# InternetMaximalism/plonky2_bn254

Hardware: AMD Instinct MI355X
Metric: G1 scalar-mul STARK proofs/sec (256-bit scalars) (higher is better)
Workload: dtype u64 (Goldilocks p = 2^64-2^32+1; BN254 Fq as 10x26-bit Montgomery limbs); 1 GPU; configs[1]: batch of 1024 G1 scalar-muls on 1 GPU per step = 8 proofs x 128 instances, 2^16 rows, W=781, standard_fast_config; instances_per_proof=128, steps_in_flight=4, parallelism=1 GPU, no collective

## Files before the change

### plonky2_bn254_amd/csrc/quotient_common.h

```cpp
#pragma once
#include "gl_dev.h"
#include "aux.h"

struct Acc {
  u64 lo, hi;
  u32 ov;
};
__device__ __forceinline__ void acc_init(Acc& a) {
  a.lo = 0;
  a.hi = 0;
  a.ov = 0;
}
__device__ __forceinline__ void acc_mad(Acc& a, u64 x, u64 w) {
  const unsigned __int128 pr = (unsigned __int128)x * w;
  u64 pl = (u64)pr, ph = (u64)(pr >> 64);
  a.lo += pl;
  u64 c = a.lo < pl ? 1 : 0;
  u64 h = a.hi + ph;
  u32 o = h < ph ? 1 : 0;
  h += c;
  o += h < c ? 1 : 0;
  a.hi = h;
  a.ov += o;
}
__device__ __forceinline__ u64 acc_red(const Acc& a) {
  return gl_sub(gl_reduce128(a.lo, a.hi), ((u64)a.ov) << 32);
}
struct Acc2 {
  Acc a0, a1;
};
__device__ __forceinline__ void acc2_init(Acc2& a) {
  acc_init(a.a0);
  acc_init(a.a1);
}
__device__ __forceinline__ void acc2_mad(Acc2& a, u64 x, u64 w0, u64 w1) {
  acc_mad(a.a0, x, w0);
  acc_mad(a.a1, x, w1);
}

static constexpr u32 M22 = (1u << 22) - 1;
struct W3 {
  u32 w0, w1, w2;
};
GL_HD W3 w3_split(u64 w) {
  W3 r;
  r.w0 = (u32)w & M22;
  r.w1 = (u32)(w >> 22) & M22;
  r.w2 = (u32)(w >> 44);
  return r;
}
struct Acc3 {
  u64 c[5];
};
__device__ __forceinline__ void acc3_init(Acc3& a) {
#pragma unroll
  for (int k = 0; k < 5; k++) a.c[k] = 0;
}
__device__ __forceinline__ void acc3_mad(Acc3& a, u32 v0, u32 v1, u32 v2, u32 w0, u32 w1, u32 w2) {
  a.c[0] += (u64)v0 * w0;
  a.c[1] += (u64)v0 * w1;
  a.c[1] += (u64)v1 * w0;
  a.c[2] += (u64)v0 * w2;
  a.c[2] += (u64)v1 * w1;
  a.c[2] += (u64)v2 * w0;
  a.c[3] += (u64)v1 * w2;
  a.c[3] += (u64)v2 * w1;
  a.c[4] += (u64)v2 * w2;
}
__device__ __forceinline__ u64 acc3_red(const Acc3& a) {
  unsigned __int128 t = (unsigned __int128)a.c[0] + ((unsigned __int128)a.c[1] << 22) + ((unsigned __int128)a.c[2] << 44);
  u64 r = gl_reduce128((u64)t, (u64)(t >> 64));
  r = gl_add(r, gl_mul_2exp<66>(gl_reduce128(a.c[3], 0)));
  r = gl_add(r, gl_mul_2exp<88>(gl_reduce128(a.c[4], 0)));
  return r;
}

struct AccW {
  Acc3 a0, a1;
};
__device__ __forceinline__ void accw_init(AccW& a) {
  acc3_init(a.a0);
  acc3_init(a.a1);
}
template <class WP>
__device__ __forceinline__ void accw_mad(AccW& a, u64 x, WP w) {
  const u32 v0 = (u32)x & M22, v1 = (u32)(x >> 22) & M22, v2 = (u32)(x >> 44);
  acc3_mad(a.a0, v0, v1, v2, w[0], w[1], w[2]);
  acc3_mad(a.a1, v0, v1, v2, w[4], w[5], w[6]);
}
GL_HD void w3_store(u64* dst , u64 wa, u64 wb) {
  const W3 a = w3_split(wa), b = w3_split(wb);
  dst[0] = (u64)a.w0 | ((u64)a.w1 << 32);
  dst[1] = (u64)a.w2;
  dst[2] = (u64)b.w0 | ((u64)b.w1 << 32);
  dst[3] = (u64)b.w2;
}

struct QPointTables {
  const u64* x;
  const u64* lfirst;
  const u64* llast;
};

__device__ __forceinline__ size_t next_position(size_t j, unsigned log_n) {
  const size_t N = (size_t)1 << log_n;
  size_t h = j >> log_n;
  u32 k = bitrev32((u32)(j & (N - 1)), log_n);
  k = (k + 1) & (u32)(N - 1);
  return (h << log_n) | bitrev32(k, log_n);
}

__device__ __forceinline__ void lookup_and_ctl_constraints(const StarkShape& sh, const u64* __restrict__ tl,
                                                           const u64* __restrict__ al, size_t M2, size_t j, size_t jn,
                                                           const u32* __restrict__ W3 , int e0,
                                                           const u64 betas[2], const u64 gammas[2], u64 lfirst, u64 llast,
                                                           u64 z_last, u64& tot0, u64& tot1) {
  const int m = sh.n_helpers(), n_rc = sh.n_rc();
  int e = e0;
  AccW acc;
  accw_init(acc);
  const u64 table = tl[(size_t)sh.table_col * M2 + j], freq = tl[(size_t)sh.freq_col * M2 + j];
  u64 hs[2] = {0, 0};
#pragma unroll 4
  for (int k = 0; k < m; k++) {
    u64 f0 = tl[(size_t)(sh.rc_begin + 2 * k) * M2 + j];
    bool two = (2 * k + 1) < n_rc;
    u64 f1 = two ? tl[(size_t)(sh.rc_begin + 2 * k + 1) * M2 + j] : 0;
#pragma unroll
    for (int ch = 0; ch < 2; ch++) {
      u64 h = al[(size_t)(ch * (m + 1) + k) * M2 + j];
      u64 g0 = gl_add(f0, betas[ch]);
      u64 c;
      if (two) {
        u64 g1 = gl_add(f1, betas[ch]);
        c = gl_sub(gl_sub(gl_mul(gl_mul(g1, g0), h), g1), g0);
      } else {
        c = gl_sub(gl_mul(g0, h), 1);
      }
      int ee = e0 + ch * (m + 2) + k;
      accw_mad(acc, c, W3 + 8 * (ee));
      hs[ch] = gl_add(hs[ch], h);
    }
  }
#pragma unroll
  for (int ch = 0; ch < 2; ch++) {
    u64 z = al[(size_t)(ch * (m + 1) + m) * M2 + j], nz = al[(size_t)(ch * (m + 1) + m) * M2 + jn];
    u64 twc = gl_add(table, betas[ch]);
    u64 y = gl_sub(gl_mul(hs[ch], twc), freq);
    int ee = e0 + ch * (m + 2) + m;
    accw_mad(acc, gl_mul(z, lfirst), W3 + 8 * (ee));
    accw_mad(acc, gl_sub(gl_mul(gl_sub(nz, z), twc), y), W3 + 8 * (ee + 1));
  }
  e = e0 + 2 * (m + 2);
  for (int ctl = 0; ctl < sh.n_ctl; ctl++) {
    u64 a0 = 0, a1 = 0;
    for (int mm = sh.ctl.ncols[ctl] - 1; mm >= 0; mm--) {
      int start = sh.ctl.col_start[ctl][mm], nb = sh.ctl.col_bits[ctl][mm];
      u64 v = 0;
      for (int b = nb - 1; b >= 0; b--) v = gl_add(gl_dbl(v), tl[(size_t)(start + b) * M2 + j]);
      a0 = gl_add(gl_mul(a0, betas[0]), v);
      a1 = gl_add(gl_mul(a1, betas[1]), v);
    }
    u64 comb[2] = {gl_add(a0, gammas[0]), gl_add(a1, gammas[1])};
    u64 f0 = tl[(size_t)sh.ctl.filter_col[ctl] * M2 + j];
#pragma unroll
    for (int ch = 0; ch < 2; ch++) {
      int zc = 2 * (m + 1) + ctl * 2 + ch;
      u64 lz = al[(size_t)zc * M2 + j], nz = al[(size_t)zc * M2 + jn];
      u64 c_last = gl_mul(gl_sub(gl_mul(comb[ch], lz), f0), llast);
      u64 c_tr = gl_mul(gl_sub(gl_mul(comb[ch], gl_sub(lz, nz)), f0), z_last);
      accw_mad(acc, c_last, W3 + 8 * (e));
      accw_mad(acc, c_tr, W3 + 8 * (e + 1));
      e += 2;
    }
  }
  tot0 = gl_add(tot0, acc3_red(acc.a0));
  tot1 = gl_add(tot1, acc3_red(acc.a1));
}
```

### plonky2_bn254_amd/csrc/quotient_g1.hip

```cpp
#include "quotient_sched.h"
#include "trace_g1.h"
#include "quotient.h"

static constexpr int G1_K_AIR = 1111;
static constexpr int G1_MZ_E0[5] = {0, 50, 83, 132, 165};

template <int part>
__device__ __forceinline__ void g1_add_part(const QArgs& A, size_t j) {
  const size_t M2 = A.stride;
  const u64* __restrict__ tl = A.tl;
  const qc64 W0 = QCONST(u64, A.W);
  const qc64 W1 = QCONST(u64, A.W + A.K);
  const qc32 W3 = QCONST(u32, A.W + 2 * (size_t)A.K);
  u64 tot0 = 0, tot1 = 0;
  int e = 0;
  const int AUX = G1_COL_AUX;
  const u64 filter = TL(G1_COL_FILTER);
  const u64 is_x_eq_filter = TL(AUX + G1_AUX_IS_X_EQ_FILTER);
  u64 ax[16], lam[16], t16[16], u16[16];
  ld16(tl, M2, j, G1_COL_A, ax);
  if constexpr (part == 0) {
    const u64 is_x_eq = TL(AUX + G1_AUX_IS_X_EQ);
    ld16(tl, M2, j, G1_COL_B, u16);
#pragma unroll
    for (int i = 0; i < 16; i++) u16[i] = gl_sub(u16[i], ax[i]);
    ld16(tl, M2, j, AUX + G1_AUX_IS_X_EQ_AUX, t16);
    const u64 c0 = gl_sub(is_x_eq, 1);
    mz_block<true>(tl, M2, j, AUX + G1_AUX_IS_X_EQ_AUX + 16, A, G1_MZ_E0[0], 0,
             filter, [&](int i) __attribute__((always_inline)) { u64 v = conv16<true>(u16, t16, i); return i == 0 ? gl_add(v, c0) : v; }, tot0, tot1);
    e = 33;
    AccW g;
    accw_init(g);
#pragma unroll
    for (int i = 0; i < 16; i++) accw_mad(g, u16[i], W3 + 8 * (e + i));
    e += 16;
    u64 f = gl_mul(filter, is_x_eq);
    tot0 = gl_add(tot0, gl_mul(f, acc3_red(g.a0)));
    tot1 = gl_add(tot1, gl_mul(f, acc3_red(g.a1)));
    EMIT(gl_sub(gl_mul(filter, is_x_eq), is_x_eq_filter));
  } else if constexpr (part == 1) {
    ld16(tl, M2, j, AUX + G1_AUX_LAMBDA, lam);
    ld16(tl, M2, j, G1_COL_B, u16);
#pragma unroll
    for (int i = 0; i < 16; i++) u16[i] = gl_sub(u16[i], ax[i]);
    ld16(tl, M2, j, G1_COL_B + 16, t16);
    ld16(tl, M2, j, G1_COL_A + 16, ax);
#pragma unroll
    for (int i = 0; i < 16; i++) t16[i] = gl_sub(t16[i], ax[i]);
    mz_block<true>(tl, M2, j, AUX + G1_AUX_LAMBDA_AUX, A, G1_MZ_E0[1], 1,
             gl_sub(filter, is_x_eq_filter),
             [&](int i) __attribute__((always_inline)) {
               u64 v = conv16<true>(lam, u16, i);
               return i < 16 ? gl_sub(v, t16[i < 16 ? i : 0]) : v;
             },
             tot0, tot1);
  } else if constexpr (part == 2) {
    ld16(tl, M2, j, AUX + G1_AUX_LAMBDA, lam);
    ld16(tl, M2, j, G1_COL_A + 16, u16);
    mz_block<true>(tl, M2, j, AUX + G1_AUX_LAMBDA_AUX, A, G1_MZ_E0[2], 2,
             is_x_eq_filter,
             [&](int i) __attribute__((always_inline)) {
               u64 ly = conv16<true>(lam, u16, i), xx = conv16<true>(ax, ax, i);
               return gl_sub(gl_dbl(ly), gl_add(gl_dbl(xx), xx));
             },
             tot0, tot1);
    e = 116;
    ld16(tl, M2, j, G1_COL_B + 16, t16);
    AccW g;
    accw_init(g);
#pragma unroll
    for (int i = 0; i < 16; i++) accw_mad(g, gl_sub(u16[i], t16[i]), W3 + 8 * (e + i));
    tot0 = gl_add(tot0, gl_mul(is_x_eq_filter, acc3_red(g.a0)));
    tot1 = gl_add(tot1, gl_mul(is_x_eq_filter, acc3_red(g.a1)));
  } else if constexpr (part == 3) {
    ld16(tl, M2, j, AUX + G1_AUX_LAMBDA, lam);
    ld16(tl, M2, j, G1_COL_B, t16);
    ld16(tl, M2, j, G1_COL_C, u16);
#pragma unroll
    for (int i = 0; i < 16; i++) ax[i] = gl_add(gl_add(ax[i], t16[i]), u16[i]);
    mz_block<true>(tl, M2, j, AUX + G1_AUX_X_AUX, A, G1_MZ_E0[3], 3, filter,
             [&](int i) __attribute__((always_inline)) {
               u64 v = conv16<true>(lam, lam, i);
               return i < 16 ? gl_sub(v, ax[i < 16 ? i : 0]) : v;
             },
             tot0, tot1);
  } else {
    ld16(tl, M2, j, AUX + G1_AUX_LAMBDA, lam);
    ld16(tl, M2, j, G1_COL_C, u16);
#pragma unroll
    for (int i = 0; i < 16; i++) u16[i] = gl_sub(u16[i], ax[i]);
    ld16(tl, M2, j, G1_COL_C + 16, t16);
    ld16(tl, M2, j, G1_COL_A + 16, ax);
#pragma unroll
    for (int i = 0; i < 16; i++) t16[i] = gl_add(t16[i], ax[i]);
    mz_block<true>(tl, M2, j, AUX + G1_AUX_Y_AUX, A, G1_MZ_E0[4], 4, filter,
             [&](int i) __attribute__((always_inline)) {
               u64 v = conv16<true>(lam, u16, i);
               return i < 16 ? gl_add(v, t16[i < 16 ? i : 0]) : v;
             },
             tot0, tot1);
  }
  store_part(A, part, j, tot0, tot1);
}

__global__ __launch_bounds__(256, 2) void k_quotient_g1_parts(QArgs A) {
  const size_t j = (size_t)blockIdx.x * blockDim.x + threadIdx.x;
  if (j >= A.count) return;
  switch (blockIdx.y) {
    case 0: schedule_part<G1L, false>(A, j, q_next(A, j), 198, 5); break;
    case 1: g1_add_part<0>(A, j); break;
    case 2: g1_add_part<1>(A, j); break;
    case 3: g1_add_part<2>(A, j); break;
    case 4: g1_add_part<3>(A, j); break;
    default: g1_add_part<4>(A, j); break;
  }
}

__global__ __launch_bounds__(256) void k_quotient_finish(QArgs A, StarkShape sh) {
  const size_t j = (size_t)blockIdx.x * blockDim.x + threadIdx.x;
  if (j >= A.count) return;
  finish_point(A, sh, j);
}
void quotient_finish_launch(const QArgs& A, const StarkShape& sh, hipStream_t st) {
  k_quotient_finish<<<(unsigned)((A.count + 255) / 256), 256, 0, st>>>(A, sh);
}

__global__ void k_point_tables(u64* x, u64* lfirst, u64* llast, unsigned log_n, u64 w_n, u64 w_2n) {
  const size_t N = (size_t)1 << log_n;
  size_t j = (size_t)blockIdx.x * blockDim.x + threadIdx.x;
  if (j >= 2 * N) return;
  size_t h = j >> log_n;
  u32 k = bitrev32((u32)(j & (N - 1)), log_n);
  u64 shift = h ? gl_mul(GL_GEN, w_2n) : GL_GEN;
  u64 xv = gl_mul(shift, gl_pow(w_n, k));
  u64 gn = gl_pow(GL_GEN, N);
  u64 zh = gl_sub(h ? gl_neg(gn) : gn, 1);
  u64 ninv = gl_inv((u64)N % GL_P);
  u64 winv = gl_inv(w_n);
  x[j] = xv;
  lfirst[j] = gl_mul(gl_mul(zh, ninv), gl_inv(gl_sub(xv, 1)));
  llast[j] = gl_mul(gl_mul(gl_mul(zh, ninv), winv), gl_inv(gl_sub(xv, winv)));
}

__global__ void k_point_tables_window(u64* x, u64* lfirst, u64* llast, unsigned log_n, u32 h, size_t k0, size_t count, u64 w_n,
                                      u64 w_2n) {
  const size_t N = (size_t)1 << log_n;
  size_t j = (size_t)blockIdx.x * blockDim.x + threadIdx.x;
  if (j >= count) return;
  const u64 k = (k0 + j) & (N - 1);
  u64 shift = h ? gl_mul(GL_GEN, w_2n) : GL_GEN;
  u64 xv = gl_mul(shift, gl_pow(w_n, k));
  u64 gn = gl_pow(GL_GEN, N);
  u64 zh = gl_sub(h ? gl_neg(gn) : gn, 1);
  u64 ninv = gl_inv((u64)N % GL_P);
  u64 winv = gl_inv(w_n);
  x[j] = xv;
  lfirst[j] = gl_mul(gl_mul(zh, ninv), gl_inv(gl_sub(xv, 1)));
  llast[j] = gl_mul(gl_mul(gl_mul(zh, ninv), winv), gl_inv(gl_sub(xv, winv)));
}
void quotient_point_tables_window(u64* d_x, u64* d_lfirst, u64* d_llast, unsigned log_n, int h, size_t k0, size_t count, hipStream_t st) {
  k_point_tables_window<<<(unsigned)((count + 255) / 256), 256, 0, st>>>(d_x, d_lfirst, d_llast, log_n, (u32)h, k0, count,
                                                                       gl_root_of_unity(log_n), gl_root_of_unity(log_n + 1));
}
void quotient_window_args(QArgs& A, const u64* d_tw, const u64* d_aw, const QPointTables& pt, u64* d_part, size_t stride, size_t count,
                          size_t k0, int h) {
  A.tl = d_tw;
  A.al = d_aw;
  A.pt = pt;
  A.part = d_part;
  A.stride = stride;
  A.count = count;
  A.k0 = k0;
  A.natural = 1;
  A.hsel = (u32)h;
}

void quotient_point_tables(u64* d_x, u64* d_lfirst, u64* d_llast, unsigned log_n, hipStream_t st) {
  size_t M2 = (size_t)2 << log_n;
  k_point_tables<<<(unsigned)((M2 + 255) / 256), 256, 0, st>>>(d_x, d_lfirst, d_llast, log_n, gl_root_of_unity(log_n),
                                                             gl_root_of_unity(log_n + 1));
}

void quotient_host_tables(int K, const u64 alphas[2], const int* mz_e0, int n_blocks, std::vector<u64>& W, std::vector<u64>& mzt) {
  W.assign(QUOTIENT_W_WORDS(K), 0);
  for (int a = 0; a < 2; a++) {
    u64 v = 1;
    for (int e = K - 1; e >= 0; e--) {
      W[(size_t)a * K + e] = v;
      v = gl_mul(v, alphas[a]);
    }
  }
  static const u64 MOD[16] = {64839, 55420, 35862, 15392, 51853, 26737, 27281, 38785,
                              22621, 33153, 17846, 47184, 41001, 57649, 20082, 12388};
  const u64 B = 1ULL << 16, OFF = 1ULL << 29;
  mzt.assign(QUOTIENT_MZT_WORDS, 0);
  for (int blk = 0; blk < n_blocks; blk++)
    for (int a = 0; a < 2; a++) {
      const u64* w = &W[(size_t)a * K + mz_e0[blk] + 1];
      u64* T = &mzt[(size_t)(blk * 2 + a) * 80];
      for (int jj = 0; jj < 17; jj++) {
        u64 s = 0;
        for (int t = 0; t < 16; t++)
          if (jj + t < 32) s = gl_add(s, gl_mul(w[jj + t], MOD[t]));
        T[jj] = s;
      }
      u64 usum = 0;
      for (int d = 0; d < 31; d++) {
        u64 u = gl_sub(w[d + 1], gl_mul(B, w[d]));
        T[17 + d] = u;
        T[48 + d] = gl_mul(B, u);
        usum = gl_add(usum, u);
      }
      T[79] = gl_mul(OFF, usum);
    }
  for (int e = 0; e < K; e++) w3_store(&W[2 * (size_t)K + 4 * (size_t)e], W[e], W[(size_t)K + e]);
  for (int blk = 0; blk < n_blocks; blk++)
    for (int t = 0; t < 80; t++)
      w3_store(&mzt[QUOTIENT_MZT3_OFF + (size_t)(blk * 80 + t) * 4], mzt[(size_t)(blk * 2) * 80 + t], mzt[(size_t)(blk * 2 + 1) * 80 + t]);
}

void quotient_fill_args(QArgs& A, const StarkShape& sh, const u64* d_tl, const u64* d_al, const u64* d_W, const u64* d_mzt,
                        const QPointTables& pt, const u64 betas[2], const u64 gammas[2], unsigned log_n, u64* d_out,
                        u64* d_part) {
  A.tl = d_tl;
  A.al = d_al;
  A.W = d_W;
  A.mzt = d_mzt;
  A.pt = pt;
  for (int i = 0; i < 2; i++) {
    A.betas[i] = betas[i];
    A.gammas[i] = gammas[i];
  }
  const size_t N = (size_t)1 << log_n;
  u64 gn = gl_pow(GL_GEN, N);
  A.zh_inv[0] = gl_inv(gl_sub(gn, 1));
  A.zh_inv[1] = gl_inv(gl_sub(gl_neg(gn), 1));
  A.w_inv = gl_inv(gl_root_of_unity(log_n));
  A.out = d_out;
  A.part = d_part;
  A.n_parts = 0;
  A.log_n = log_n;
  A.K = sh.n_total_constraints();
  A.stride = A.count = 2 * N;
  A.k0 = 0;
  A.natural = 0;
  A.hsel = 0;
}

int g1_quotient_mz_blocks(const int** e0) {
  *e0 = G1_MZ_E0;
  return 5;
}
void g1_quotient_launch(const QArgs& A0, const StarkShape& sh, hipStream_t st) {
  QArgs A = A0;
  A.n_parts = 6;
  const unsigned g = (unsigned)((A.count + 255) / 256);
  k_quotient_g1_parts<<<dim3(g, 6), 256, 0, st>>>(A);
  quotient_finish_launch(A, sh, st);
}

void quotient_g1_module_warm() {
  hipFuncAttributes a;
  (void)hipFuncGetAttributes(&a, reinterpret_cast<const void*>(&k_point_tables));
}
```

### plonky2_bn254_amd/csrc/quotient_g2fq.hip

```cpp
#include "quotient_sched.h"
#include "quotient.h"

static constexpr int G2_MZ_E0[10] = {1, 50, 100, 133, 166, 199, 264, 297, 330, 363};
static constexpr int FQ_MZ_E0[1] = {0};

__device__ __forceinline__ u64 econv_c0(const u64* x0, const u64* x1, const u64* y0, const u64* y1, int i) {
  return gl_sub(conv16(x0, y0, i), conv16(x1, y1, i));
}
__device__ __forceinline__ u64 econv_c1(const u64* x0, const u64* x1, const u64* y0, const u64* y1, int i) {
  return gl_add(conv16(x0, y1, i), conv16(x1, y0, i));
}

#define MZB(blk, auxcol, FILTER, FN, ...) \
  mz_block(tl, M2, j, (auxcol), A, G2_MZ_E0[blk], (blk), (FILTER), FN, tot0, tot1, ##__VA_ARGS__)

__global__ __launch_bounds__(256, 2) void k_quotient_g2_sched(QArgs A) {
  const size_t j = (size_t)blockIdx.x * blockDim.x + threadIdx.x;
  if (j >= A.count) return;
  schedule_part<G2L, false>(A, j, q_next(A, j), 396, 6);
}

template <int part>
__global__ __launch_bounds__(256, 2) void k_quotient_g2_add(QArgs A) {
  typedef G2L L;
  const size_t M2 = A.stride;
  const size_t j = (size_t)blockIdx.x * blockDim.x + threadIdx.x;
  if (j >= A.count) return;
  const u64* __restrict__ tl = A.tl;
  const qc64 W0 = QCONST(u64, A.W);
  const qc64 W1 = QCONST(u64, A.W + A.K);
  const qc32 W3 = QCONST(u32, A.W + 2 * (size_t)A.K);
  u64 tot0 = 0, tot1 = 0;
  int e = 0;
  const u64 filter = TL(L::FILTER);
  const int AUX = L::AUX;
  u64 is_x_eq_filter = 0;
  if constexpr (part == 1 || part == 2) is_x_eq_filter = TL(AUX + G2_AUX_IS_X_EQ_FILTER);
  auto seed_w = [&](Acc2& sd, int blk, int i, u64 v) { acc2_mad(sd, v, W0[G2_MZ_E0[blk] + 1 + i], W1[G2_MZ_E0[blk] + 1 + i]); };
  if constexpr (part == 0 || part == 5) {
    constexpr int h = part == 0 ? 0 : 1;
    u64 dx[16], t0[16];
    const u64 z = TL(AUX + (h ? G2_AUX_IS_C1_ZERO : G2_AUX_IS_C0_ZERO));
    if constexpr (h == 0) {
      EMIT(gl_mul(filter, gl_sub(gl_mul(z, TL(AUX + G2_AUX_IS_C1_ZERO)), TL(AUX + G2_AUX_IS_X_EQ))));
    }
#pragma unroll
    for (int i = 0; i < 16; i++) dx[i] = gl_sub(TL(L::B + 16 * h + i), TL(L::A + 16 * h + i));
    ld16(tl, M2, j, AUX + (h ? G2_AUX_C1_AUX : G2_AUX_C0_AUX), t0);
    const u64 c0 = gl_sub(z, 1);
    MZB(h, AUX + (h ? G2_AUX_C1_AUX : G2_AUX_C0_AUX) + 16, filter, [&](int i) __attribute__((always_inline)) { u64 v = conv16(dx, t0, i); return i == 0 ? gl_add(v, c0) : v; });
    e = h ? 83 : 34;
    AccW g;
    accw_init(g);
#pragma unroll
    for (int i = 0; i < 16; i++) accw_mad(g, dx[i], W3 + 8 * (e + i));
    const u64 f = gl_mul(filter, z);
    tot0 = gl_add(tot0, gl_mul(f, acc3_red(g.a0)));
    tot1 = gl_add(tot1, gl_mul(f, acc3_red(g.a1)));
    if constexpr (h == 1) {
      e = 99;
      EMIT(gl_sub(gl_mul(filter, TL(AUX + G2_AUX_IS_X_EQ)), TL(AUX + G2_AUX_IS_X_EQ_FILTER)));
    }
  } else {
    Acc2 sd0, sd1;
    acc2_init(sd0);
    acc2_init(sd1);
    u64 l0[16], l1[16], dx0[16], dx1[16];
    if constexpr (part == 1) {
#pragma unroll 4
      for (int i = 0; i < 16; i++) seed_w(sd0, 2, i, gl_sub(TL(L::A + 32 + i), TL(L::B + 32 + i)));
      ld16(tl, M2, j, AUX + G2_AUX_LAMBDA, l0);
      ld16(tl, M2, j, AUX + G2_AUX_LAMBDA + 16, l1);
#pragma unroll
      for (int i = 0; i < 16; i++) {
        dx0[i] = gl_sub(TL(L::B + i), TL(L::A + i));
        dx1[i] = gl_sub(TL(L::B + 16 + i), TL(L::A + 16 + i));
      }
      const u64 f_ne = gl_sub(filter, is_x_eq_filter);
      MZB(2, AUX + G2_AUX_LAMBDA_AUX, f_ne, [&](int i) __attribute__((always_inline)) { return econv_c0(l0, l1, dx0, dx1, i); }, &sd0);
#pragma unroll 4
      for (int i = 0; i < 16; i++) seed_w(sd1, 3, i, gl_sub(TL(L::A + 48 + i), TL(L::B + 48 + i)));
      MZB(3, AUX + G2_AUX_LAMBDA_AUX + 80, f_ne, [&](int i) __attribute__((always_inline)) { return econv_c1(l0, l1, dx0, dx1, i); }, &sd1);
    } else if constexpr (part == 2) {
      ld16(tl, M2, j, L::A, dx0);
      ld16(tl, M2, j, L::A + 16, dx1);
#pragma unroll
      for (int i = 0; i < 31; i++) {
        const u64 xx0 = econv_c0(dx0, dx1, dx0, dx1, i), xx1 = econv_c1(dx0, dx1, dx0, dx1, i);
        seed_w(sd0, 4, i, gl_neg(gl_add(gl_dbl(xx0), xx0)));
        seed_w(sd1, 5, i, gl_neg(gl_add(gl_dbl(xx1), xx1)));
      }
      ld16(tl, M2, j, AUX + G2_AUX_LAMBDA, l0);
      ld16(tl, M2, j, AUX + G2_AUX_LAMBDA + 16, l1);
      ld16(tl, M2, j, L::A + 32, dx0);
      ld16(tl, M2, j, L::A + 48, dx1);
      MZB(4, AUX + G2_AUX_LAMBDA_AUX, is_x_eq_filter, [&](int i) __attribute__((always_inline)) { return gl_dbl(econv_c0(l0, l1, dx0, dx1, i)); }, &sd0);
      MZB(5, AUX + G2_AUX_LAMBDA_AUX + 80, is_x_eq_filter, [&](int i) __attribute__((always_inline)) { return gl_dbl(econv_c1(l0, l1, dx0, dx1, i)); }, &sd1);
      e = 232;
      AccW g;
      accw_init(g);
#pragma unroll
      for (int i = 0; i < 16; i++) accw_mad(g, gl_sub(dx0[i], TL(L::B + 32 + i)), W3 + 8 * (e + i));
#pragma unroll
      for (int i = 0; i < 16; i++) accw_mad(g, gl_sub(dx1[i], TL(L::B + 48 + i)), W3 + 8 * (e + 16 + i));
      tot0 = gl_add(tot0, gl_mul(is_x_eq_filter, acc3_red(g.a0)));
      tot1 = gl_add(tot1, gl_mul(is_x_eq_filter, acc3_red(g.a1)));
    } else if constexpr (part == 3) {
#pragma unroll 4
      for (int i = 0; i < 16; i++) {
        seed_w(sd0, 6, i, gl_neg(gl_add(gl_add(TL(L::A + i), TL(L::B + i)), TL(L::C + i))));
        seed_w(sd1, 7, i, gl_neg(gl_add(gl_add(TL(L::A + 16 + i), TL(L::B + 16 + i)), TL(L::C + 16 + i))));
      }
      ld16(tl, M2, j, AUX + G2_AUX_LAMBDA, l0);
      ld16(tl, M2, j, AUX + G2_AUX_LAMBDA + 16, l1);
      MZB(6, AUX + G2_AUX_X_AUX, filter, [&](int i) __attribute__((always_inline)) { return econv_c0(l0, l1, l0, l1, i); }, &sd0);
      MZB(7, AUX + G2_AUX_X_AUX + 80, filter, [&](int i) __attribute__((always_inline)) { return econv_c1(l0, l1, l0, l1, i); }, &sd1);
    } else {
#pragma unroll 4
      for (int i = 0; i < 16; i++) seed_w(sd0, 8, i, gl_add(TL(L::C + 32 + i), TL(L::A + 32 + i)));
      ld16(tl, M2, j, AUX + G2_AUX_LAMBDA, l0);
      ld16(tl, M2, j, AUX + G2_AUX_LAMBDA + 16, l1);
#pragma unroll
      for (int i = 0; i < 16; i++) {
        dx0[i] = gl_sub(TL(L::C + i), TL(L::A + i));
        dx1[i] = gl_sub(TL(L::C + 16 + i), TL(L::A + 16 + i));
      }
      MZB(8, AUX + G2_AUX_Y_AUX, filter, [&](int i) __attribute__((always_inline)) { return econv_c0(l0, l1, dx0, dx1, i); }, &sd0);
#pragma unroll 4
      for (int i = 0; i < 16; i++) seed_w(sd1, 9, i, gl_add(TL(L::C + 48 + i), TL(L::A + 48 + i)));
      MZB(9, AUX + G2_AUX_Y_AUX + 80, filter, [&](int i) __attribute__((always_inline)) { return econv_c1(l0, l1, dx0, dx1, i); }, &sd1);
    }
  }
  store_part(A, part, j, tot0, tot1);
}

__global__ __launch_bounds__(256, 2) void k_quotient_fq_sched(QArgs A) {
  const size_t j = (size_t)blockIdx.x * blockDim.x + threadIdx.x;
  if (j >= A.count) return;
  schedule_part<FQL, true>(A, j, q_next(A, j), 33, 1);
}
__global__ __launch_bounds__(256) void k_quotient_fq_mul(QArgs A) {
  typedef FQL L;
  const size_t M2 = A.stride;
  const size_t j = (size_t)blockIdx.x * blockDim.x + threadIdx.x;
  if (j >= A.count) return;
  const u64* __restrict__ tl = A.tl;
  const qc64 W0 = QCONST(u64, A.W);
  const qc64 W1 = QCONST(u64, A.W + A.K);
  u64 tot0 = 0, tot1 = 0;
  const u64 filter = TL(L::FILTER);
  u64 a[16], b[16], c[16];
  ld16(tl, M2, j, L::A, a);
  ld16(tl, M2, j, L::B, b);
  ld16(tl, M2, j, L::C, c);
  mz_block(tl, M2, j, L::AUX, A, FQ_MZ_E0[0], 0, filter,
           [&](int i) __attribute__((always_inline)) {
             u64 v = conv16(a, b, i);
             return i < 16 ? gl_sub(v, c[i < 16 ? i : 0]) : v;
           },
           tot0, tot1);
  store_part(A, 0, j, tot0, tot1);
}

int g2_quotient_mz_blocks(const int** e0) {
  *e0 = G2_MZ_E0;
  return 10;
}
int fq_quotient_mz_blocks(const int** e0) {
  *e0 = FQ_MZ_E0;
  return 1;
}
void g2_quotient_launch(const QArgs& A0, const StarkShape& sh, hipStream_t st) {
  QArgs A = A0;
  A.n_parts = 7;
  const unsigned g = (unsigned)((A.count + 255) / 256);
  k_quotient_g2_add<0><<<g, 256, 0, st>>>(A);
  k_quotient_g2_add<5><<<g, 256, 0, st>>>(A);
  k_quotient_g2_add<1><<<g, 256, 0, st>>>(A);
  k_quotient_g2_add<2><<<g, 256, 0, st>>>(A);
  k_quotient_g2_add<3><<<g, 256, 0, st>>>(A);
  k_quotient_g2_add<4><<<g, 256, 0, st>>>(A);
  k_quotient_g2_sched<<<g, 256, 0, st>>>(A);
  quotient_finish_launch(A, sh, st);
}
void fq_quotient_launch(const QArgs& A0, const StarkShape& sh, hipStream_t st) {
  QArgs A = A0;
  A.n_parts = 2;
  const unsigned g = (unsigned)((A.count + 255) / 256);
  k_quotient_fq_mul<<<g, 256, 0, st>>>(A);
  k_quotient_fq_sched<<<g, 256, 0, st>>>(A);
  quotient_finish_launch(A, sh, st);
}

void quotient_g2fq_module_warm() {
  hipFuncAttributes a;
  (void)hipFuncGetAttributes(&a, reinterpret_cast<const void*>(&k_quotient_fq_sched));
}
```

### plonky2_bn254_amd/csrc/quotient_sched.h

```cpp
#pragma once
#include <vector>
#include "quotient_common.h"
#include "layout.h"

#ifndef MZ_CONSTS
#define MZ_CONSTS
static constexpr int QMZ_IQP = 0, QMZ_QUOT = 1, QMZ_LO = 18, QMZ_HI = 49;
#endif

struct QArgs {
  const u64* tl;
  const u64* al;
  const u64* W;
  const u64* mzt;
  QPointTables pt;
  u64 betas[2], gammas[2];
  u64 zh_inv[2];
  u64 w_inv;
  u64* out;
  u64* part;
  int n_parts;
  unsigned log_n;
  int K;
  size_t stride, count, k0;
  u32 natural, hsel;
};
static constexpr size_t QUOTIENT_MZT3_OFF = 10 * 2 * 80, QUOTIENT_MZT_WORDS = 10 * 2 * 80 + 10 * 80 * 4;
static inline size_t QUOTIENT_W_WORDS(int K) { return 6 * (size_t)K; }
__device__ __forceinline__ size_t q_next(const QArgs& A, size_t j) { return A.natural ? j + 1 : next_position(j, A.log_n); }

#define QCONST(T, p) ((const __attribute__((address_space(4))) T*)(p))
typedef const __attribute__((address_space(4))) u64* qc64;
typedef const __attribute__((address_space(4))) u32* qc32;

#define TL(c) tl[(size_t)(c)*M2 + j]
#define TN(c) tl[(size_t)(c)*M2 + jn]

__device__ __forceinline__ void ld16(const u64* __restrict__ tl, size_t M2, size_t j, int col, u64* v) {
#pragma unroll
  for (int i = 0; i < 16; i++) v[i] = tl[(size_t)(col + i) * M2 + j];
}
template <bool FULL = false>
__device__ __forceinline__ u64 conv16(const u64* A, const u64* B, int i) {
  Acc a;
  acc_init(a);
  if constexpr (FULL) {
#pragma clang loop unroll(full)
    for (int s = 0; s < 16; s++) {
      int t = i - s;
      if (t >= 0 && t < 16) acc_mad(a, A[s], B[t]);
    }
  } else {
#pragma unroll
    for (int s = 0; s < 16; s++) {
      int t = i - s;
      if (t >= 0 && t < 16) acc_mad(a, A[s], B[t]);
    }
  }
  return acc_red(a);
}

template <bool FULL = false, class InFn>
__device__ __forceinline__ void mz_block(const u64* __restrict__ tl, size_t M2, size_t j, int auxcol, const QArgs& A, int e0, int blk,
                                         u64 filter, InFn in, u64& tot0, u64& tot1, const Acc2* seed = nullptr) {
  const qc64 w0 = QCONST(u64, A.W + e0);
  const qc64 w1 = QCONST(u64, A.W + A.K + e0);
  const qc64 T0 = QCONST(u64, A.mzt + (size_t)blk * 160);
  const qc64 T1 = T0 + 80;
  const qc32 w3 = QCONST(u32, A.W + 2 * (size_t)A.K) + 8 * (size_t)e0;
  const qc32 T3 = QCONST(u32, A.mzt + QUOTIENT_MZT3_OFF) + 8 * (size_t)(blk * 80);
  u64 n0, n1;
  {
    Acc2 neg;
    if (seed) neg = *seed;
    else acc2_init(neg);
    if constexpr (FULL) {
#pragma clang loop unroll(full)
      for (int i = 0; i < 31; i++) {
        acc2_mad(neg, in(i), w0[1 + i], w1[1 + i]);
        if (i % 8 == 7) {
          asm volatile("" : "+v"(neg.a0.lo), "+v"(neg.a0.hi), "+v"(neg.a0.ov), "+v"(neg.a1.lo), "+v"(neg.a1.hi), "+v"(neg.a1.ov));
          __builtin_amdgcn_sched_barrier(0);
        }
      }
    } else {
#pragma unroll
      for (int i = 0; i < 31; i++) {
        acc2_mad(neg, in(i), w0[1 + i], w1[1 + i]);
        __builtin_amdgcn_sched_barrier(0);
      }
    }
    n0 = acc_red(neg.a0);
    n1 = acc_red(neg.a1);
    asm volatile("" : "+v"(n0), "+v"(n1));
  }
  __builtin_amdgcn_sched_barrier(0);
  const u64 iqp = TL(auxcol + QMZ_IQP);
  const u64 qsign = gl_sub(gl_dbl(iqp), 1);
  u64 s0, s1;
  {
    AccW q;
    accw_init(q);
#pragma unroll 1
    for (int jj = 0; jj < 17; jj++) accw_mad(q, TL(auxcol + QMZ_QUOT + jj), T3 + 8 * jj);
    s0 = gl_mul(qsign, acc3_red(q.a0));
    s1 = gl_mul(qsign, acc3_red(q.a1));
  }
  __builtin_amdgcn_sched_barrier(0);
  {
    AccW pos;
    accw_init(pos);
    accw_mad(pos, gl_sub(gl_mul(iqp, iqp), iqp), w3);
#pragma unroll 1
    for (int d = 0; d < 31; d++) {
      accw_mad(pos, TL(auxcol + QMZ_LO + d), T3 + 8 * (17 + d));
      accw_mad(pos, TL(auxcol + QMZ_HI + d), T3 + 8 * (48 + d));
    }
    s0 = gl_add(s0, acc3_red(pos.a0));
    s1 = gl_add(s1, acc3_red(pos.a1));
  }
  s0 = gl_sub(gl_sub(s0, T0[79]), n0);
  s1 = gl_sub(gl_sub(s1, T1[79]), n1);
  tot0 = gl_add(tot0, gl_mul(filter, s0));
  tot1 = gl_add(tot1, gl_mul(filter, s1));
  asm volatile("" : "+v"(tot0), "+v"(tot1));
}

#define EQ_GROUP(filter, n, AEXPR, BEXPR)                         \
  {                                                               \
    static_assert((n) % 16 == 0, "EQ_GROUP: n % 16");             \
    AccW g_;                                                      \
    accw_init(g_);                                                \
    constexpr int CH_ = 16;                                       \
    _Pragma("unroll 1") for (int i0_ = 0; i0_ < (n); i0_ += CH_) { \
      u64 d_[CH_];                                                \
      _Pragma("unroll") for (int k_ = 0; k_ < CH_; k_++) {        \
        const int i = i0_ + k_;                                   \
        d_[k_] = gl_sub((AEXPR), (BEXPR));                        \
      }                                                           \
      _Pragma("unroll") for (int k_ = 0; k_ < CH_; k_++) accw_mad(g_, d_[k_], W3 + 8 * (e + i0_ + k_)); \
    }                                                             \
    e += (n);                                                     \
    u64 f_ = (filter);                                            \
    tot0 = gl_add(tot0, gl_mul(f_, acc3_red(g_.a0)));             \
    tot1 = gl_add(tot1, gl_mul(f_, acc3_red(g_.a1)));             \
    asm volatile("" : "+v"(tot0), "+v"(tot1));  \
  }
#define EMIT(c)                                  \
  {                                              \
    u64 c_ = (c);                                \
    tot0 = gl_add(tot0, gl_mul(c_, W0[e]));      \
    tot1 = gl_add(tot1, gl_mul(c_, W1[e]));      \
    e += 1;                                      \
  }


__device__ __forceinline__ void store_part(const QArgs& A, int part, size_t j, u64 tot0, u64 tot1) {
  const size_t M2 = A.stride;
  A.part[((size_t)part * 2 + 0) * M2 + j] = tot0;
  A.part[((size_t)part * 2 + 1) * M2 + j] = tot1;
}

template <class L, bool FIRST_A_IS_ONE>
__device__ __forceinline__ void schedule_part(const QArgs& A, size_t j, size_t jn, int e, int part) {
  u64 tot0 = 0, tot1 = 0;
  const size_t M2 = A.stride;
  const u64* __restrict__ tl = A.tl;
  const qc64 W0 = QCONST(u64, A.W);
  const qc64 W1 = QCONST(u64, A.W + A.K);
  const qc32 W3 = QCONST(u32, A.W + 2 * (size_t)A.K);
  const u64 filter = TL(L::FILTER);
  const u64 is_first = TL(L::FLAGS + 0), is_last = TL(L::FLAGS + 1);
  const u64 n_filter = TN(L::FILTER), n_is_last = TN(L::FLAGS + 1);
  const u64 is_not_last_round = gl_sub(filter, is_last);
  const u64 is_next_not_last_round = gl_sub(n_filter, n_is_last);
  const u64 is_adding = TL(L::IS_ADDING), idnl = TL(L::IDNL);
  const u64 n_is_adding = TN(L::IS_ADDING), n_idnl = TN(L::IDNL);
  const u64 bit0 = TL(L::BITS), n_bit0 = TN(L::BITS);

  EMIT(gl_mul(is_first, gl_sub(is_adding, 1)));
  EQ_GROUP(is_first, L::PL, TL(L::DOUBLE + i), TL(L::B + i));
  EQ_GROUP(gl_mul(bit0, is_first), L::PL, TL(L::SUM + i), TL(L::C + i));
  EQ_GROUP(gl_mul(gl_sub(1, bit0), is_first), L::PL, TL(L::SUM + i), TL(L::A + i));
  if (FIRST_A_IS_ONE) {
    EQ_GROUP(is_first, L::PL, TL(L::A + i), (u64)(i == 0 ? 1 : 0));
  }
  EQ_GROUP(idnl, L::PL, TN(L::A + i), TL(L::SUM + i));
  EQ_GROUP(idnl, L::PL, TN(L::B + i), TL(L::DOUBLE + i));
  EQ_GROUP(gl_mul(n_bit0, idnl), L::PL, TN(L::SUM + i), TN(L::C + i));
  EQ_GROUP(gl_mul(gl_sub(1, n_bit0), idnl), L::PL, TN(L::SUM + i), TN(L::A + i));
  EQ_GROUP(idnl, L::PL, TN(L::DOUBLE + i), TL(L::DOUBLE + i));
  EMIT(gl_mul(idnl, gl_sub(n_is_adding, 1)));
  EMIT(gl_mul(idnl, n_idnl));
  EQ_GROUP(idnl, 256, TN(L::BITS + i), TL(L::BITS + ((i + 1) & 255)));
  EQ_GROUP(is_adding, L::PL, TN(L::A + i), TL(L::DOUBLE + i));
  EQ_GROUP(is_adding, L::PL, TN(L::B + i), TL(L::DOUBLE + i));
  EQ_GROUP(is_adding, L::PL, TN(L::SUM + i), TL(L::SUM + i));
  EQ_GROUP(is_adding, L::PL, TN(L::DOUBLE + i), TN(L::C + i));
  EMIT(gl_mul(is_adding, n_is_adding));
  EMIT(gl_mul(is_adding, gl_sub(n_idnl, is_next_not_last_round)));
  EQ_GROUP(is_adding, 256, TN(L::BITS + i), TL(L::BITS + i));
  {
    const u64 counter = TL(L::FLAGS + 2), inv_c = TL(L::FLAGS + 3), inv_cp = TL(L::FLAGS + 4);
    const u64 n_counter = TN(L::FLAGS + 2);
    const u64 not_filter = gl_sub(1, filter);
    EMIT(gl_mul(not_filter, is_first));
    EMIT(gl_mul(not_filter, is_last));
    EMIT(gl_mul(filter, gl_sub(gl_mul(counter, inv_c), gl_sub(1, is_first))));
    EMIT(gl_mul(gl_mul(filter, counter), is_first));
    const u64 cp = gl_sub(counter, 511);
    EMIT(gl_mul(filter, gl_sub(gl_mul(cp, inv_cp), gl_sub(1, is_last))));
    EMIT(gl_mul(gl_mul(filter, cp), is_last));
    EMIT(gl_mul(gl_mul(filter, gl_sub(1, is_last)), gl_sub(gl_sub(n_counter, counter), 1)));
    EMIT(gl_mul(gl_mul(filter, is_last), n_counter));
  }
  EMIT(gl_mul(is_not_last_round, gl_sub(TN(L::TIMESTAMP), TL(L::TIMESTAMP))));
  EMIT(gl_mul(is_not_last_round, gl_sub(n_filter, filter)));
  const u64 x = A.pt.x[j], llast = A.pt.llast[j];
  const u64 z_last = gl_sub(x, A.w_inv);
  {
    const u64 rc = TL(L::RANGE), diff = gl_sub(TN(L::RANGE), rc);
    EMIT(gl_mul(gl_sub(gl_mul(diff, diff), diff), z_last));
    EMIT(gl_mul(gl_sub(rc, 65535), llast));
  }
  store_part(A, part, j, tot0, tot1);
}

__device__ __forceinline__ void finish_point(const QArgs& A, const StarkShape& sh, size_t j) {
  const unsigned log_n = A.log_n;
  const size_t N = (size_t)1 << log_n, M2 = A.stride;
  const size_t jn = q_next(A, j);
  u64 tot0 = 0, tot1 = 0;
  for (int p = 0; p < A.n_parts; p++) {
    tot0 = gl_add(tot0, A.part[((size_t)p * 2 + 0) * M2 + j]);
    tot1 = gl_add(tot1, A.part[((size_t)p * 2 + 1) * M2 + j]);
  }
  const u64 x = A.pt.x[j], lfirst = A.pt.lfirst[j], llast = A.pt.llast[j];
  const u64 z_last = gl_sub(x, A.w_inv);
  lookup_and_ctl_constraints(sh, A.tl, A.al, M2, j, jn, (const u32*)(A.W + 2 * (size_t)A.K), sh.n_constraints, A.betas, A.gammas,
                             lfirst, llast, z_last, tot0, tot1);
  const size_t h = A.natural ? A.hsel : j >> log_n;
  const size_t k = A.natural ? A.k0 + j : (size_t)bitrev32((u32)(j & (N - 1)), log_n);
  A.out[(0 * 2 + h) * N + k] = gl_mul(tot0, A.zh_inv[h]);
  A.out[(1 * 2 + h) * N + k] = gl_mul(tot1, A.zh_inv[h]);
}

void quotient_host_tables(int K, const u64 alphas[2], const int* mz_e0, int n_blocks, std::vector<u64>& W, std::vector<u64>& mzt);
void quotient_fill_args(QArgs& A, const StarkShape& sh, const u64* d_tl, const u64* d_al, const u64* d_W, const u64* d_mzt,
                        const QPointTables& pt, const u64 betas[2], const u64 gammas[2], unsigned log_n, u64* d_out,
                        u64* d_part);
static constexpr int QUOTIENT_MAX_PARTS = 7;
void quotient_finish_launch(const QArgs& A, const StarkShape& sh, hipStream_t st);
```

Measured before the change: 92.56 proofs/s.

## Split lookup helper constraints into parallel slice kernels before quotient finish

Moves the range-check lookup helper constraint evaluation out of the serial finish kernel into separate slices, run as extra grid rows of the G1 parts kernel or as a dedicated launch for G2/Fq. Each slice writes partial constraint sums and helper sums to part buffers, which finish_point then accumulates before evaluating the Z and CTL constraints. This spreads the heavy helper loop across more threads and blocks, at the cost of extra part-buffer traffic and, for G2/Fq, one more kernel launch. It also uses a variant Goldilocks multiply (gl_mul_rep) in the helper loop.

```diff
diff --git a/plonky2_bn254_amd/csrc/quotient_common.h b/plonky2_bn254_amd/csrc/quotient_common.h
--- a/plonky2_bn254_amd/csrc/quotient_common.h
+++ b/plonky2_bn254_amd/csrc/quotient_common.h
@@ -110,22 +110,31 @@
   return (h << log_n) | bitrev32(k, log_n);
 }
 
-__device__ __forceinline__ void lookup_and_ctl_constraints(const StarkShape& sh, const u64* __restrict__ tl,
-                                                           const u64* __restrict__ al, size_t M2, size_t j, size_t jn,
-                                                           const u32* __restrict__ W3 , int e0,
-                                                           const u64 betas[2], const u64 gammas[2], u64 lfirst, u64 llast,
-                                                           u64 z_last, u64& tot0, u64& tot1) {
-  const int m = sh.n_helpers(), n_rc = sh.n_rc();
-  int e = e0;
+__device__ __forceinline__ u64 gl_mul_rep(u64 a, u64 b) {
+  const unsigned __int128 x = (unsigned __int128)a * b;
+  const u64 lo = (u64)x, hi = (u64)(x >> 64);
+  const u64 hi_hi = hi >> 32, hi_lo = hi & GL_EPS;
+  u64 t0 = lo - hi_hi;
+  t0 = (lo < hi_hi) ? t0 - GL_EPS : t0;
+  const u64 t1 = (hi_lo << 32) - hi_lo;
+  const u64 r = t0 + t1;
+  return r < t1 ? r + GL_EPS : r;
+}
+
+template <class WP>
+__device__ __forceinline__ void lookup_helper_constraints(const u64* __restrict__ tl, const u64* __restrict__ al, size_t M2, size_t j,
+                                                          WP W3 , int e0, int rc_begin, int n_rc,
+                                                          int k_begin, int k_end, const u64 betas[2], u64& tot0, u64& tot1,
+                                                          u64 hs[2]) {
+  const int m = (n_rc + 1) / 2;
   AccW acc;
   accw_init(acc);
-  const u64 table = tl[(size_t)sh.table_col * M2 + j], freq = tl[(size_t)sh.freq_col * M2 + j];
-  u64 hs[2] = {0, 0};
+  hs[0] = hs[1] = 0;
 #pragma unroll 4
-  for (int k = 0; k < m; k++) {
-    u64 f0 = tl[(size_t)(sh.rc_begin + 2 * k) * M2 + j];
+  for (int k = k_begin; k < k_end; k++) {
+    u64 f0 = tl[(size_t)(rc_begin + 2 * k) * M2 + j];
     bool two = (2 * k + 1) < n_rc;
-    u64 f1 = two ? tl[(size_t)(sh.rc_begin + 2 * k + 1) * M2 + j] : 0;
+    u64 f1 = two ? tl[(size_t)(rc_begin + 2 * k + 1) * M2 + j] : 0;
 #pragma unroll
     for (int ch = 0; ch < 2; ch++) {
       u64 h = al[(size_t)(ch * (m + 1) + k) * M2 + j];
@@ -133,15 +142,27 @@
       u64 c;
       if (two) {
         u64 g1 = gl_add(f1, betas[ch]);
-        c = gl_sub(gl_sub(gl_mul(gl_mul(g1, g0), h), g1), g0);
+        c = gl_sub(gl_sub(gl_mul_rep(gl_mul_rep(g1, g0), h), g1), g0);
       } else {
-        c = gl_sub(gl_mul(g0, h), 1);
+        c = gl_sub(gl_mul_rep(g0, h), 1);
       }
-      int ee = e0 + ch * (m + 2) + k;
-      accw_mad(acc, c, W3 + 8 * (ee));
+      accw_mad(acc, c, W3 + 8 * (e0 + ch * (m + 2) + k));
       hs[ch] = gl_add(hs[ch], h);
     }
   }
+  tot0 = acc3_red(acc.a0);
+  tot1 = acc3_red(acc.a1);
+}
+
+template <class WP>
+__device__ __forceinline__ void z_and_ctl_constraints(const StarkShape& sh, const u64* __restrict__ tl, const u64* __restrict__ al,
+                                                      size_t M2, size_t j, size_t jn, WP W3 , int e0,
+                                                      const u64 betas[2], const u64 gammas[2], const u64 hs[2], u64 lfirst,
+                                                      u64 llast, u64 z_last, u64& tot0, u64& tot1) {
+  const int m = sh.n_helpers();
+  AccW acc;
+  accw_init(acc);
+  const u64 table = tl[(size_t)sh.table_col * M2 + j], freq = tl[(size_t)sh.freq_col * M2 + j];
 #pragma unroll
   for (int ch = 0; ch < 2; ch++) {
     u64 z = al[(size_t)(ch * (m + 1) + m) * M2 + j], nz = al[(size_t)(ch * (m + 1) + m) * M2 + jn];
@@ -151,7 +172,7 @@
     accw_mad(acc, gl_mul(z, lfirst), W3 + 8 * (ee));
     accw_mad(acc, gl_sub(gl_mul(gl_sub(nz, z), twc), y), W3 + 8 * (ee + 1));
   }
-  e = e0 + 2 * (m + 2);
+  int e = e0 + 2 * (m + 2);
   for (int ctl = 0; ctl < sh.n_ctl; ctl++) {
     u64 a0 = 0, a1 = 0;
     for (int mm = sh.ctl.ncols[ctl] - 1; mm >= 0; mm--) {
diff --git a/plonky2_bn254_amd/csrc/quotient_g1.hip b/plonky2_bn254_amd/csrc/quotient_g1.hip
--- a/plonky2_bn254_amd/csrc/quotient_g1.hip
+++ b/plonky2_bn254_amd/csrc/quotient_g1.hip
@@ -112,8 +112,18 @@
     case 2: g1_add_part<1>(A, j); break;
     case 3: g1_add_part<2>(A, j); break;
     case 4: g1_add_part<3>(A, j); break;
-    default: g1_add_part<4>(A, j); break;
-  }
+    case 5: g1_add_part<4>(A, j); break;
+    default: lookup_slice_part(A, j, (int)blockIdx.y - 6); break;
+  }
+}
+
+__global__ __launch_bounds__(256) void k_quotient_lookup_parts(QArgs A) {
+  const size_t j = (size_t)blockIdx.x * blockDim.x + threadIdx.x;
+  if (j >= A.count) return;
+  lookup_slice_part(A, j, (int)blockIdx.y);
+}
+void quotient_lookup_launch(const QArgs& A, hipStream_t st) {
+  k_quotient_lookup_parts<<<dim3((unsigned)((A.count + 255) / 256), QUOTIENT_LOOKUP_SLICES), 256, 0, st>>>(A);
 }
 
 __global__ __launch_bounds__(256) void k_quotient_finish(QArgs A, StarkShape sh) {
@@ -239,6 +249,9 @@
   A.out = d_out;
   A.part = d_part;
   A.n_parts = 0;
+  A.rc_begin = sh.rc_begin;
+  A.n_rc = sh.n_rc();
+  A.e_lookup = sh.n_constraints;
   A.log_n = log_n;
   A.K = sh.n_total_constraints();
   A.stride = A.count = 2 * N;
@@ -255,7 +268,7 @@
   QArgs A = A0;
   A.n_parts = 6;
   const unsigned g = (unsigned)((A.count + 255) / 256);
-  k_quotient_g1_parts<<<dim3(g, 6), 256, 0, st>>>(A);
+  k_quotient_g1_parts<<<dim3(g, 6 + QUOTIENT_LOOKUP_SLICES), 256, 0, st>>>(A);
   quotient_finish_launch(A, sh, st);
 }
 
diff --git a/plonky2_bn254_amd/csrc/quotient_g2fq.hip b/plonky2_bn254_amd/csrc/quotient_g2fq.hip
--- a/plonky2_bn254_amd/csrc/quotient_g2fq.hip
+++ b/plonky2_bn254_amd/csrc/quotient_g2fq.hip
@@ -181,6 +181,7 @@
   k_quotient_g2_add<3><<<g, 256, 0, st>>>(A);
   k_quotient_g2_add<4><<<g, 256, 0, st>>>(A);
   k_quotient_g2_sched<<<g, 256, 0, st>>>(A);
+  quotient_lookup_launch(A, st);
   quotient_finish_launch(A, sh, st);
 }
 void fq_quotient_launch(const QArgs& A0, const StarkShape& sh, hipStream_t st) {
@@ -189,6 +190,7 @@
   const unsigned g = (unsigned)((A.count + 255) / 256);
   k_quotient_fq_mul<<<g, 256, 0, st>>>(A);
   k_quotient_fq_sched<<<g, 256, 0, st>>>(A);
+  quotient_lookup_launch(A, st);
   quotient_finish_launch(A, sh, st);
 }
 
diff --git a/plonky2_bn254_amd/csrc/quotient_sched.h b/plonky2_bn254_amd/csrc/quotient_sched.h
--- a/plonky2_bn254_amd/csrc/quotient_sched.h
+++ b/plonky2_bn254_amd/csrc/quotient_sched.h
@@ -20,6 +20,8 @@
   u64* out;
   u64* part;
   int n_parts;
+  int rc_begin, n_rc;
+  int e_lookup;
   unsigned log_n;
   int K;
   size_t stride, count, k0;
@@ -226,19 +228,38 @@
   store_part(A, part, j, tot0, tot1);
 }
 
+static constexpr int QUOTIENT_LOOKUP_SLICES = 2;
+__device__ __forceinline__ void lookup_slice_part(const QArgs& A, size_t j, int slice) {
+  const int m = (A.n_rc + 1) / 2, per = (m + QUOTIENT_LOOKUP_SLICES - 1) / QUOTIENT_LOOKUP_SLICES;
+  const int k_begin = min(m, slice * per), k_end = min(m, k_begin + per);
+  u64 tot0, tot1, hs[2];
+  lookup_helper_constraints(A.tl, A.al, A.stride, j, QCONST(u32, A.W + 2 * (size_t)A.K), A.e_lookup, A.rc_begin, A.n_rc, k_begin, k_end,
+                            A.betas, tot0, tot1, hs);
+  store_part(A, A.n_parts + 2 * slice, j, tot0, tot1);
+  store_part(A, A.n_parts + 2 * slice + 1, j, hs[0], hs[1]);
+}
+
 __device__ __forceinline__ void finish_point(const QArgs& A, const StarkShape& sh, size_t j) {
   const unsigned log_n = A.log_n;
   const size_t N = (size_t)1 << log_n, M2 = A.stride;
   const size_t jn = q_next(A, j);
-  u64 tot0 = 0, tot1 = 0;
+  u64 tot0 = 0, tot1 = 0, hs[2] = {0, 0};
   for (int p = 0; p < A.n_parts; p++) {
     tot0 = gl_add(tot0, A.part[((size_t)p * 2 + 0) * M2 + j]);
     tot1 = gl_add(tot1, A.part[((size_t)p * 2 + 1) * M2 + j]);
   }
+#pragma unroll
+  for (int s = 0; s < QUOTIENT_LOOKUP_SLICES; s++) {
+    const size_t p = (size_t)A.n_parts + 2 * s;
+    tot0 = gl_add(tot0, A.part[(p * 2 + 0) * M2 + j]);
+    tot1 = gl_add(tot1, A.part[(p * 2 + 1) * M2 + j]);
+    hs[0] = gl_add(hs[0], A.part[(p * 2 + 2) * M2 + j]);
+    hs[1] = gl_add(hs[1], A.part[(p * 2 + 3) * M2 + j]);
+  }
   const u64 x = A.pt.x[j], lfirst = A.pt.lfirst[j], llast = A.pt.llast[j];
   const u64 z_last = gl_sub(x, A.w_inv);
-  lookup_and_ctl_constraints(sh, A.tl, A.al, M2, j, jn, (const u32*)(A.W + 2 * (size_t)A.K), sh.n_constraints, A.betas, A.gammas,
-                             lfirst, llast, z_last, tot0, tot1);
+  z_and_ctl_constraints(sh, A.tl, A.al, M2, j, jn, QCONST(u32, A.W + 2 * (size_t)A.K), sh.n_constraints, A.betas, A.gammas, hs, lfirst,
+                        llast, z_last, tot0, tot1);
   const size_t h = A.natural ? A.hsel : j >> log_n;
   const size_t k = A.natural ? A.k0 + j : (size_t)bitrev32((u32)(j & (N - 1)), log_n);
   A.out[(0 * 2 + h) * N + k] = gl_mul(tot0, A.zh_inv[h]);
@@ -249,5 +270,6 @@
 void quotient_fill_args(QArgs& A, const StarkShape& sh, const u64* d_tl, const u64* d_al, const u64* d_W, const u64* d_mzt,
                         const QPointTables& pt, const u64 betas[2], const u64 gammas[2], unsigned log_n, u64* d_out,
                         u64* d_part);
-static constexpr int QUOTIENT_MAX_PARTS = 7;
+static constexpr int QUOTIENT_MAX_PARTS = 7 + 2 * QUOTIENT_LOOKUP_SLICES;
+void quotient_lookup_launch(const QArgs& A, hipStream_t st);
 void quotient_finish_launch(const QArgs& A, const StarkShape& sh, hipStream_t st);
```

Result: slower. 90.75 proofs/s (-2.0%).
